# NVIDIA-Merlin/Transformers4Rec

Hardware: AMD Instinct MI355X
Metric: training sessions/sec (XLNet 4x128, 100k items, seq 20, MLM, tied full softmax) + Recall@20 (higher is better)
Workload: dtype f32; 1 GPU; BASELINE.json configs[1]: synthetic schema, item vocab 100k (100001 table rows), d_model 128, 4-layer 4-head XLNet, seq_len 20, per-GPU batch 1024, MLM p=0.15, tied-weight full softmax, Adam, fwd+bwd+gradient exchange+optimizer per step; global_batch=1024, seq_len=20, parallelism=dp1, head_mode=materialize, precision_mode=auto, table_exchange=local, world_size=1, gpu_max_hw_queues=4, extra_streams=0, prefetch=1, preheat_steps=1847

## Files before the change

### transformers4rec_amd/_lib.py

```python
import ctypes
import os
import re

_HERE = os.path.dirname(os.path.abspath(__file__))
LIB_PATH = os.environ.get("T4R_HIP_LIB") or os.path.join(_HERE, "lib", "libt4r_hip.so")
HEADER_PATH = os.path.join(os.path.dirname(_HERE), "include", "t4r_hip.h")
SAMPLING_HEADER_PATH = os.path.join(os.path.dirname(_HERE), "include", "t4r_hip_sampling.h")
FILTER_HEADER_PATH = os.path.join(os.path.dirname(_HERE), "include", "t4r_hip_filter.h")
OPTIM_HEADER_PATH = os.path.join(os.path.dirname(_HERE), "include", "t4r_hip_optim.h")
PRETRAINED_HEADER_PATH = os.path.join(os.path.dirname(_HERE), "include", "t4r_hip_pretrained.h")
ATTN_HEADER_PATH = os.path.join(os.path.dirname(_HERE), "include", "t4r_hip_attn.h")
ROWS_HEADER_PATH = os.path.join(os.path.dirname(_HERE), "include", "t4r_hip_rows.h")
ROWADAM_HEADER_PATH = os.path.join(os.path.dirname(_HERE), "include", "t4r_hip_rowadam.h")
CONTPROJ_HEADER_PATH = os.path.join(os.path.dirname(_HERE), "include", "t4r_hip_contproj.h")
ROWCLIP_HEADER_PATH = os.path.join(os.path.dirname(_HERE), "include", "t4r_hip_rowclip.h")

_P, _I, _L, _F, _Q = ctypes.c_void_p, ctypes.c_int, ctypes.c_long, ctypes.c_float, ctypes.c_ulonglong
_C = {"p": _P, "i": _I, "l": _L, "f": _F, "Q": _Q}

_SIGS = {
    "t4r_abi_version": ("i", ""),
    "t4r_last_error": ("s", ""),
    "t4r_ragged_max_len": ("i", "ppip"),
    "t4r_ragged_to_padded": ("i", "ppppiii"),
    "t4r_ragged_gather_to_padded": ("i", "pppp" + "p" + "iii"),
    "t4r_seq_features_fwd": ("i", "pippppppiiiiiiipppp"),
    "t4r_embedding_bwd": ("i", "pppp" + "liiilii"),
    "t4r_sort_ids_ws_bytes": ("l", "l"),
    "t4r_sort_ids": ("i", "pp" + "lli" + "ppp" + "l"),
    "t4r_sort_ids_multi_ws_bytes": ("l", "li"),
    "t4r_sort_ids_multi": ("i", "ppilpp" + "ppp" + "l"),
    "t4r_embedding_bwd_sorted_ws_floats": ("l", "li"),
    "t4r_embedding_bwd_sorted": ("i", "ppppp" + "liiili" + "p"),
    "t4r_embedding_bag_fwd": ("i", "pp" + "li" + "pp" + "llii" + "p" + "li" + "p"),
    "t4r_embedding_bag_bwd_rows": ("i", "pp" + "lii" + "p" + "llii" + "p"),
    "t4r_apply_mask_fwd": ("i", "ppppiiii"),
    "t4r_apply_mask_bwd": ("i", "ppppiiii" + "p"),
    "t4r_apply_mask_bwd_ws_floats": ("l", "iii"),
    "t4r_apply_mask_bwd_to": ("i", "pppppiiii" + "p"),
    "t4r_mul": ("i", "ppppl"),
    "t4r_soft_embedding_fwd": ("i", "pppppppp" + "liif"),
    "t4r_soft_embedding_bwd": ("i", "pppppppppppp" + "liiiif" + "p"),
    "t4r_soft_embedding_bwd_ws_floats": ("l", "lii"),
    "t4r_mask_targets": ("i", "ppiiil" + "ppp" + "fQQ" + "ppp"),
    "t4r_compact_labels": ("i", "pppiil" + "pppp"),
    "t4r_gather_rows": ("i", "ppppii"),
    "t4r_scatter_rows_add": ("i", "ppppii"),
    "t4r_scatter_rows_dense": ("i", "pppippli"),
    "t4r_last_positions": ("i", "ppiiiilp"),
    "t4r_gemm_f32": ("i", "piiiiif" + "plplpl" + "pipl" + "iii" + "lll" + "fQQ"),
    "t4r_gemm_splitk_sink_begin": ("v", "pl"),
    "t4r_gemm_splitk_sink_flush": ("i", "p"),
    "t4r_gemm_splitk_sink_end": ("v", ""),
    "t4r_gemm_splitk_sink_bypassed": ("i", ""),
    "t4r_mha_fwd": ("i", "pppplplp" + "iiiii" + "fQQ" + "p"),
    "t4r_mha_bwd": ("i", "pppplpplppppl" + "iiiii" + "fQQ" + "p"),
    "t4r_add_pos_fwd": ("i", "ppppp" + "iii"),
    "t4r_add_pos_bwd": ("i", "ppp" + "iii"),
    "t4r_dropout_ctr_hi": ("Q", "Qii"),
    "t4r_dropout": ("i", "pppp" + "llfQQ"),
    "t4r_set_precision": ("v", "i"),
    "t4r_get_precision": ("i", ""),
    "t4r_gemm_softmax_grad_f32": ("i", "piiiif" + "plpppf" + "plpl" + "ii"),
    "t4r_set_tok_gemm_min_rows": ("v", "i"),
    "t4r_get_tok_gemm_min_rows": ("i", ""),
    "t4r_head_split_supported": ("i", "i"),
    "t4r_head_split_fwd_products": ("i", ""),
    "t4r_head_split_ws_bytes": ("l", "iii"),
    "t4r_head_split_prepare": ("i", "ppl" + "iii" + "p"),
    "t4r_head_split_fdx_supported": ("i", "i"),
    "t4r_head_split_logits_ce_dx": ("i", "pp" + "plpl" + "pl" + "pppp" + "plp" + "iii" + "ff" + "p"),
    "t4r_head_note_dw_form": ("i", "p"),
    "t4r_head_split_logits": ("i", "ppplpl" + "iiif" + "p"),
    "t4r_head_split_logits_ce": ("i", "ppplpl" + "pppp" + "iiiff" + "p"),
    "t4r_head_split_dw": ("i", "ppplpppf" + "pl" + "iiiii" + "fi" + "p"),
    "t4r_head_split_dx": ("i", "ppplpppf" + "plpl" + "iiiii" + "fi" + "p"),
    "t4r_head_split_recompute_supported": ("i", "i"),
    "t4r_head_split_prepare_rc": ("i", "ppl" + "iii" + "p"),
    "t4r_head_split_ce": ("i", "ppplpppp" + "iiiff" + "p"),
    "t4r_head_split_dw_rc": ("i", "ppplpppf" + "pl" + "iiifi" + "p"),
    "t4r_head_split_dx_rc": ("i", "ppplplpppf" + "pl" + "iiifi" + "p"),
    "t4r_add_layernorm_fwd": ("i", "pppppppp" + "iif" + "fQQ"),
    "t4r_add_layernorm_bwd": ("i", "pppppppppppp" + "iii" + "fQQ"),
    "t4r_colreduce_ws_floats": ("l", "li"),
    "t4r_act_bwd_bias": ("i", "pppppp" + "lii" + "fQQ"),
    "t4r_colsum": ("i", "pppp" + "lil"),
    "t4r_session_lengths": ("i", "pp" + "iiii" + "p"),
    "t4r_xlnet_attn_fwd": ("i", "ppppppppp" + "iiii" + "ifQQ" + "p"),
    "t4r_xlnet_attn_bwd_ws_floats": ("l", "iiii"),
    "t4r_xlnet_attn_bwd": ("i", "p" * 17 + "iiii" + "ifQQ" + "p"),
    "t4r_xlnet_fused_supported": ("i", "i"),
    "t4r_xlnet_fused_products": ("i", ""),
    "t4r_xlnet_ff_bwd_part_floats": ("l", "li"),
    "t4r_xlnet_layer_planes_floats": ("l", "i"),
    "t4r_xlnet_layer_prepare": ("i", "ppip"),
    "t4r_xlnet_qkv_proj": ("i", "pppp" + "li"),
    "t4r_xlnet_kr_proj": ("i", "pppp" + "li"),
    "t4r_xlnet_oproj_ln": ("i", "p" + "ppppp" + "pppp" + "liff" + "QQ"),
    "t4r_xlnet_ln1_bwd_part_floats": ("l", "li"),
    "t4r_xlnet_ln1_bwd": ("i", "p" + "ppppppp" + "pppppp" + "lif" + "QQ"),
    "t4r_xlnet_dh": ("i", "pppp" + "li"),
    "t4r_xlnet_set_cu_budget": ("v", "i"),
    "t4r_xlnet_get_cu_budget": ("i", ""),
    "t4r_device_cus": ("i", ""),
    "t4r_experimental_build": ("i", ""),
    "t4r_xlnet_attn_block_supported": ("i", "iii"),
    "t4r_xlnet_attn_block_fwd": ("i", "ppppp" + "l" + "pppp" + "ppppppp" + "iiii" + "ffQQQ" + "p"),
    "t4r_xlnet_layer_bwd_defer": ("v", "i"),
    "t4r_xlnet_layer_ws_offsets": ("i", "iiiii" + "pp"),
    "t4r_xlnet_stack_prepare": ("i", "ppiip" + "plp"),
    "t4r_xlnet_stack_pos_dropout": ("v", "fQQlp"),
    "t4r_xlnet_stack_prepared": ("v", "i"),
    "t4r_xlnet_layer_bwd_join": ("i", "p"),
    "t4r_xlnet_ff_planes_floats": ("l", "i"),
    "t4r_xlnet_ff_prepare": ("i", "ppppip"),
    "t4r_xlnet_ff_fwd": ("i", "p" + "pppppp" + "pppppp" + "iiff" + "QQQ"),
    "t4r_xlnet_ff_bwd": ("i", "p" + "pppppppp" + "pppppppp" + "iif" + "QQQ"),
    "t4r_xlnet_layer_ws_floats": ("l", "iiiii"),
    "t4r_xlnet_layer_bwd_ws_floats": ("l", "iiiii"),
    "t4r_xlnet_layer_fwd": ("i", "pppppp" + "iiiif" + "fQQi" + "pp"),
    "t4r_xlnet_layer_bwd": ("i", "ppppppppp" + "iiiif" + "fQQi" + "pp"),
    "t4r_softmax_ce_fwd": ("i", "pppppp" + "iilf"),
    "t4r_softmax_ce_bwd": ("i", "pppppp" + "iilf"),
    "t4r_linear_softmax_ce_chunk_floats": ("l", "ii"),
    "t4r_linear_softmax_ce_fwd": ("i", "pplpl" + "p" + "iiiffi" + "ppppp"),
    "t4r_linear_softmax_ce_bwd": ("i", "pplpl" + "ppp" + "iiiffi" + "pplpl"),
    "t4r_sampled_logits_fwd": ("i", "ppppppp" + "iiif" + "p"),
    "t4r_log_uniform_sample": ("i", "pp" + "ill" + "QQ"),
    "t4r_sampled_logits_bwd": ("i", "ppppppppp" + "iiif"),
    "t4r_sampled_logits_bwd_rows": ("i", "ppppppppp" + "iiif"),
    "t4r_topk": ("i", "pp" + "iili" + "pp"),
    "t4r_rank_of_target_f32": ("i", "p" + "iiif" + "pl" + "pl" + "ppp"),
    "t4r_item_topk_ws_bytes": ("l", "iiii"),
    "t4r_item_topk_f32": ("i", "p" + "iiif" + "pl" + "pl" + "i" + "pp" + "pl" + "p"),
    "t4r_item_table_image_ld": ("i", "i"),
    "t4r_item_topk_h16_supported": ("i", "i"),
    "t4r_item_table_pack_h16": ("i", "p" + "pl" + "iii" + "pl"),
    "t4r_item_scores_h16": ("i", "p" + "iiif" + "pl" + "pl" + "i" + "pl" + "pl"),
    "t4r_item_topk_h16_ws_bytes": ("l", "iiii"),
    "t4r_item_topk_h16": ("i", "p" + "iiif" + "pl" + "pl" + "i" + "i" + "pp" + "pl" + "p"),
    "t4r_item_eval_h16_ws_bytes": ("l", "iii"),
    "t4r_item_eval_h16": ("i", "p" + "iiif" + "pl" + "pl" + "i" + "p" + "pppp" + "pl"),
    "t4r_swap_noise_ws_bytes": ("l", "l"),
    "t4r_swap_noise": ("i", "ppp" + "il" + "pllf" + "pp" + "QQ" + "pl"),
    "t4r_copy_cols": ("i", "pp" + "li" + "p" + "ili"),
    "t4r_seq_sum_cols": ("i", "pp" + "li" + "p" + "ili"),
    "t4r_adam_step": ("i", "ppppp" + "li" + "ffffff" + "i"),
    "t4r_adam_step_amax": ("i", "ppppp" + "li" + "ffffff" + "i" + "llp"),
    "t4r_head_split_w_amax_hint": ("v", "ppi"),
}

_SIGS_SAMPLING = {
    "t4r_gumbel_add_f32": ("i", "pp" + "iill" + "i" + "QQ"),
    "t4r_gumbel_argmax_f32": ("i", "pp" + "iill" + "QQ" + "pp"),
    "t4r_item_sample_ws_bytes": ("l", "iiii"),
    "t4r_item_sample_f32": ("i", "p" + "iiif" + "pl" + "pl" + "i" + "pp" + "pl" + "p" + "lQQ"),
    "t4r_item_sample_h16_ws_bytes": ("l", "iiii"),
    "t4r_item_sample_h16": ("i", "p" + "iiif" + "pl" + "pl" + "i" + "i" + "pp" + "pl" + "p" + "lQQ"),
}

_FILT = "ppil"
_SIGS_FILTER = {
    "t4r_item_allow_words": ("l", "i"),
    "t4r_item_allow_pack": ("i", "ppip"),
    "t4r_item_mask_f32": ("i", "pp" + "iili" + _FILT),
    "t4r_item_topk_filtered_f32": ("i", _SIGS["t4r_item_topk_f32"][1] + _FILT),
    "t4r_item_topk_filtered_h16": ("i", _SIGS["t4r_item_topk_h16"][1] + _FILT),
    "t4r_item_sample_filtered_f32": ("i", _SIGS_SAMPLING["t4r_item_sample_f32"][1] + _FILT),
    "t4r_item_sample_filtered_h16": ("i", _SIGS_SAMPLING["t4r_item_sample_h16"][1] + _FILT),
}

_SIGS_OPTIM = {
    "t4r_grad_sumsq_parts": ("l", "l"),
    "t4r_grad_sumsq": ("i", "pplp"),
    "t4r_grad_clip_coef": ("i", "ppiffp"),
    "t4r_adamw_step": ("i", "ppppp" + "li" + "fffff" + "if" + "i" + "p" + "llp"),
}

_PP = "pipllpli"
_SIGS_PRETRAINED = {
    "t4r_pretrained_proj_ws_bytes": ("l", "ii"),
    "t4r_pretrained_proj_fwd": ("i", _PP + "ppppfii" + "pli" + "pppp"),
    "t4r_pretrained_proj_bwd_ws_floats": ("l", "lii"),
    "t4r_pretrained_proj_bwd": ("i", _PP + "pli" + "ppp" + "ii" + "ppppp"),
}

_SIGS_ATTN = {
    "t4r_xlnet_attn_block_fwd_prob": ("i", "ppppp" + "l" + "pppp" + "pppppppp" + "iiii" + "ffQQQ" + "p"),
    "t4r_xlnet_attn_bwd_prob": ("i", "p" * 16 + "iiii" + "ifQQ"),
}

_SIGS_ROWS = {
    "t4r_xlnet_ff_fwd_rows": ("i", _SIGS["t4r_xlnet_ff_fwd"][1] + "pi"),
    "t4r_xlnet_ff_bwd_rows": ("i", _SIGS["t4r_xlnet_ff_bwd"][1] + "pip"),
    "t4r_xlnet_ln1_bwd_rows": ("i", "p" + "ppppppp" + "ppp" + "ppp" + "lif" + "QQ" + "pi"),
    "t4r_xlnet_layer_fwd_rows": ("i", _SIGS["t4r_xlnet_layer_fwd"][1] + "pi"),
    "t4r_xlnet_layer_bwd_rows": ("i", _SIGS["t4r_xlnet_layer_bwd"][1] + "pi"),
}

_SIGS_ROWADAM = {
    "t4r_row_adam_ws_bytes": ("l", "li"),
    "t4r_row_adam_step": ("i", "pppp" + "li" + "ppp" + "lli" + "fffff" + "if" + "pl"),
}

_CP = "pp" + "liii" + "pp"
_SIGS_CONTPROJ = {
    "t4r_cont_proj_supported": ("i", "ii"),
    "t4r_cont_proj_bwd_ws_floats": ("l", "lii"),
    "t4r_cont_proj_fwd": ("i", "p" + _CP + "p"),
    "t4r_cont_proj_bwd": ("i", "p" + "pli" + _CP + "pppp"),
}

_SIGS_ROWCLIP = {
    "t4r_row_grad_sumsq_parts": ("l", "li"),
    "t4r_row_adam_reduce": ("i", "pli" + "ppp" + "ll" + "pl" + "p"),
    "t4r_row_adam_apply": ("i", "pppp" + "li" + "li" + "fffff" + "if" + "p" + "pl"),
}

_lib = None


class T4RHipError(RuntimeError):
    pass


def _declared(path):
    with open(path) as f:
        text = re.sub(r"/\*.*?\*/", "", f.read(), flags=re.S)
    return sorted(set(re.findall(r"\b(t4r_\w+)\s*\(", text)))


def header_symbols():
    return _declared(HEADER_PATH)


def sampling_header_symbols():
    return _declared(SAMPLING_HEADER_PATH)


def filter_header_symbols():
    return _declared(FILTER_HEADER_PATH)


def optim_header_symbols():
    return _declared(OPTIM_HEADER_PATH)


def pretrained_header_symbols():
    return _declared(PRETRAINED_HEADER_PATH)


def attn_header_symbols():
    return _declared(ATTN_HEADER_PATH)


def rows_header_symbols():
    return _declared(ROWS_HEADER_PATH)


def rowadam_header_symbols():
    return _declared(ROWADAM_HEADER_PATH)


def contproj_header_symbols():
    return _declared(CONTPROJ_HEADER_PATH)


def rowclip_header_symbols():
    return _declared(ROWCLIP_HEADER_PATH)


def load():
    global _lib
    if _lib is not None:
        return _lib
    if not os.path.exists(LIB_PATH):
        raise T4RHipError(
            f"{LIB_PATH} not found: the HIP extension is not built "
            "(run `python -m transformers4rec_amd.build`). There is no CPU fallback.")
    lib = ctypes.CDLL(LIB_PATH)
    for name, (ret, args) in (list(_SIGS.items()) + list(_SIGS_SAMPLING.items()) + list(_SIGS_FILTER.items()) + list(_SIGS_OPTIM.items())
                              + list(_SIGS_PRETRAINED.items()) + list(_SIGS_ATTN.items()) + list(_SIGS_ROWS.items()) + list(_SIGS_ROWADAM.items())
                              + list(_SIGS_CONTPROJ.items()) + list(_SIGS_ROWCLIP.items())):
        fn = getattr(lib, name)
        fn.restype = ctypes.c_char_p if ret == "s" else (None if ret == "v" else _C[ret])
        fn.argtypes = [_C[a] for a in args]
    _lib = lib
    return lib


def check(rc, what):
    if rc != 0:
        msg = load().t4r_last_error()
        raise T4RHipError(f"{what} failed (rc={rc}): {msg.decode() if msg else ''}")


def call(name, *args):
    rc = getattr(load(), name)(*args)
    if rc != 0:
        check(rc, name)


def ptr_array(ptrs):
    arr = (ctypes.c_void_p * len(ptrs))(*ptrs)
    return ctypes.cast(arr, ctypes.c_void_p), arr


def int_array(vals):
    arr = (ctypes.c_int * len(vals))(*vals)
    return ctypes.cast(arr, ctypes.c_void_p), arr


def long_array(vals):
    arr = (ctypes.c_long * len(vals))(*vals)
    return ctypes.cast(arr, ctypes.c_void_p), arr


def exp_env(name, default=None):
    v = os.environ.get(name)
    if v is None:
        return default
    try:
        return v if load().t4r_experimental_build() else default
    except Exception:
        return default
```

### transformers4rec_amd/csrc/embedding_sorted.hip

```cpp
#include "t4r_common.h"
#include "seg_sum_kernel.h"
#include <hipcub/hipcub.hpp>

static size_t al256(size_t b) { return (b + 255) & ~(size_t)255; }

__global__ __launch_bounds__(256) void emb_keys_kernel(const long* __restrict__ ids, long n, long rows,
                                                        int padding_idx, int* __restrict__ keys,
                                                        int* __restrict__ idx) {
    const long i = (long)blockIdx.x * blockDim.x + threadIdx.x;
    if (i >= n) return;
    const long id = ids[i];
    keys[i] = (id == padding_idx || id < 0 || id >= rows) ? (int)rows : (int)id;
    idx[i] = (int)i;
}

struct SortLayout { size_t keys_in, idx_in, tmp, tmp_bytes, total; };
static SortLayout sort_layout(long n) {
    SortLayout l;
    size_t o = 0;
    auto take = [&](size_t b) { size_t at = o; o += al256(b); return at; };
    l.keys_in = take((size_t)n * 4);
    l.idx_in = take((size_t)n * 4);
    size_t sb = 0;
    (void)hipcub::DeviceRadixSort::SortPairs(nullptr, sb, (int*)nullptr, (int*)nullptr, (int*)nullptr,
                                             (int*)nullptr, (int)n);
    l.tmp_bytes = sb;
    l.tmp = take(sb);
    l.total = o;
    return l;
}

extern "C" long t4r_sort_ids_ws_bytes(long n) { return n <= 0 ? 0 : (long)sort_layout(n).total; }

extern "C" int t4r_sort_ids(void* stream, const long* ids, long n, long rows, int padding_idx,
                            int* keys_sorted, int* perm, void* ws, long ws_bytes) {
    if (n <= 0) return 0;
    T4R_CHECK_ARG(ids && keys_sorted && perm && ws, "sort_ids: null pointer");
    T4R_CHECK_ARG(n < (1L << 31) && rows > 0 && rows < (1L << 31) - 1, "sort_ids: sizes must fit 31 bits");
    const SortLayout l = sort_layout(n);
    T4R_CHECK_ARG(ws_bytes >= (long)l.total, "sort_ids: workspace too small (t4r_sort_ids_ws_bytes)");
    hipStream_t st = (hipStream_t)stream;
    char* w = (char*)ws;
    int* keys_in = (int*)(w + l.keys_in);
    int* idx_in = (int*)(w + l.idx_in);
    hipLaunchKernelGGL(emb_keys_kernel, dim3((unsigned)((n + 255) / 256)), dim3(256), 0, st, ids, n, rows,
                       padding_idx, keys_in, idx_in);
    int end_bit = 1;
    while (end_bit < 31 && (1L << end_bit) <= rows) ++end_bit;
    size_t tb = l.tmp_bytes;
    if (hipcub::DeviceRadixSort::SortPairs(w + l.tmp, tb, keys_in, keys_sorted, idx_in, perm, (int)n, 0, end_bit,
                                           st) != hipSuccess) {
        t4r_set_error("sort_ids: device radix sort failed");
        return -1;
    }
    T4R_LAUNCH_CHECK();
    return 0;
}

constexpr int kSortMaxFeatures = 16;
struct SortMulti { const long* ids[kSortMaxFeatures]; long rows[kSortMaxFeatures]; long off[kSortMaxFeatures]; int pad[kSortMaxFeatures]; int F; long n; };

__global__ __launch_bounds__(256) void emb_keys_multi_kernel(SortMulti p, int* __restrict__ keys, int* __restrict__ idx) {
    const long i = (long)blockIdx.x * blockDim.x + threadIdx.x;
    if (i >= p.n * p.F) return;
    const int f = (int)(i / p.n);
    const long id = p.ids[f][i - f * p.n];
    const long rows = p.rows[f];
    keys[i] = (int)(p.off[f] + ((id == p.pad[f] || id < 0 || id >= rows) ? rows : id));
    idx[i] = (int)i;
}
__global__ __launch_bounds__(256) void emb_keys_multi_fix_kernel(SortMulti p, int* __restrict__ keys, int* __restrict__ perm) {
    const long i = (long)blockIdx.x * blockDim.x + threadIdx.x;
    if (i >= p.n * p.F) return;
    const int f = (int)(i / p.n);
    keys[i] -= (int)p.off[f];
    perm[i] -= (int)(f * p.n);
}

extern "C" long t4r_sort_ids_multi_ws_bytes(long n, int F) { return (n <= 0 || F <= 0) ? 0 : (long)sort_layout(n * F).total; }

extern "C" int t4r_sort_ids_multi(void* stream, const long* const* ids, int F, long n, const long* rows, const int* padding_idx,
                                  int* keys_sorted, int* perm, void* ws, long ws_bytes) {
    if (n <= 0 || F <= 0) return 0;
    T4R_CHECK_ARG(ids && rows && padding_idx && keys_sorted && perm && ws, "sort_ids_multi: null pointer");
    T4R_CHECK_ARG(F <= kSortMaxFeatures, "sort_ids_multi: at most 16 tables per call");
    SortMulti p;
    p.F = F; p.n = n;
    long off = 0;
    for (int f = 0; f < F; ++f) {
        T4R_CHECK_ARG(ids[f] && rows[f] > 0, "sort_ids_multi: null ids or empty table");
        p.ids[f] = ids[f]; p.rows[f] = rows[f]; p.pad[f] = padding_idx[f]; p.off[f] = off;
        off += rows[f] + 1;
    }
    T4R_CHECK_ARG(n * F < (1L << 31) && off < (1L << 31) - 1, "sort_ids_multi: sizes must fit 31 bits");
    const SortLayout l = sort_layout(n * F);
    T4R_CHECK_ARG(ws_bytes >= (long)l.total, "sort_ids_multi: workspace too small (t4r_sort_ids_multi_ws_bytes)");
    hipStream_t st = (hipStream_t)stream;
    char* w = (char*)ws;
    int* keys_in = (int*)(w + l.keys_in);
    int* idx_in = (int*)(w + l.idx_in);
    const unsigned grid = (unsigned)((n * F + 255) / 256);
    hipLaunchKernelGGL(emb_keys_multi_kernel, dim3(grid), dim3(256), 0, st, p, keys_in, idx_in);
    int end_bit = 1;
    while (end_bit < 31 && (1L << end_bit) < off) ++end_bit;
    size_t tb = l.tmp_bytes;
    if (hipcub::DeviceRadixSort::SortPairs(w + l.tmp, tb, keys_in, keys_sorted, idx_in, perm, (int)(n * F), 0, end_bit, st) !=
        hipSuccess) {
        t4r_set_error("sort_ids_multi: device radix sort failed");
        return -1;
    }
    hipLaunchKernelGGL(emb_keys_multi_fix_kernel, dim3(grid), dim3(256), 0, st, p, keys_sorted, perm);
    T4R_LAUNCH_CHECK();
    return 0;
}

extern "C" long t4r_embedding_bwd_sorted_ws_floats(long n, int dim) { return seg_ws_floats(n, dim); }

extern "C" int t4r_embedding_bwd_sorted(void* stream, const float* dout, const int* keys_sorted,
                                        const int* perm, float* dtable, long n, int W, int col, int dim,
                                        long rows, int ids_div, float* ws) {
    if (n <= 0) return 0;
    T4R_CHECK_ARG(dout && keys_sorted && perm && dtable && ws, "embedding_bwd_sorted: null pointer");
    T4R_CHECK_ARG(ids_div >= 1 && dim >= 1 && col >= 0 && col + dim <= W, "embedding_bwd_sorted: bad slice");
    T4R_CHECK_ARG(rows < (1L << 31) - 1, "embedding_bwd_sorted: rows must fit 31 bits");
    seg_sum_launch<false>((hipStream_t)stream, dout, keys_sorted, perm, dtable, ws, n, W, col, dim, (int)rows, ids_div);
    T4R_LAUNCH_CHECK();
    return 0;
}
```

### transformers4rec_amd/features.py

```python
import functools
import math
import os
from typing import Dict, Optional

import torch
from torch import nn

from . import ops
from .transformations import TabularDropout, TabularLayerNorm, parse_post, parse_pre
from .masking import MaskSequence, _grad_buf, parse_masking
from .schema import Tags, categorical_cardinalities



def _table_scatter(ctx, name, grad_rows, ids_f, tab, col, dim, padding_idx):
    ids_div = grad_rows.numel() // grad_rows.shape[-1] // ids_f.numel()
    sink = getattr(tab, "_t4r_sparse_sink", None)
    if sink is not None:
        sink.add(tab, ids_f, grad_rows, col, dim, ids_div, padding_idx)
        return
    srt = ctx.sorted_ids.get(name)
    if srt is None:
        srt = ops.sort_ids(ids_f, tab.shape[0], padding_idx)
    ops.embedding_bwd_sorted(grad_rows, srt[0], srt[1], _grad_buf(tab), col, dim, ids_div)


def _sort_ids_forward(ids, rows, padding_idx):
    return ops.sort_ids(ids, rows, padding_idx)


def _sort_ids_forward_multi(ids_list, rows_list, padding_idx):
    return ops.sort_ids_multi(ids_list, rows_list, [padding_idx] * len(ids_list))


class EmbeddingTable(nn.Module):

    def __init__(self, num_embeddings, embedding_dim, padding_idx=None, std=0.05):
        super().__init__()
        self.num_embeddings, self.embedding_dim, self.padding_idx = num_embeddings, embedding_dim, padding_idx
        self.weight = nn.Parameter(torch.empty(num_embeddings, embedding_dim))
        nn.init.normal_(self.weight, mean=0.0, std=std)

    def extra_repr(self):
        return f"{self.num_embeddings}, {self.embedding_dim}, padding_idx={self.padding_idx}"


class _Linear(nn.Module):

    def __init__(self, in_features, out_features, bias=True):
        super().__init__()
        self.in_features, self.out_features = in_features, out_features
        self.weight = nn.Parameter(torch.empty(out_features, in_features))
        self.bias = nn.Parameter(torch.empty(out_features)) if bias else None
        nn.init.kaiming_uniform_(self.weight, a=math.sqrt(5))
        if bias:
            bound = 1 / math.sqrt(in_features) if in_features > 0 else 0
            nn.init.uniform_(self.bias, -bound, bound)


class _LayerNormParams(nn.Module):
    def __init__(self, dim, eps=1e-5):
        super().__init__()
        self.eps = eps
        self.weight = nn.Parameter(torch.ones(dim))
        self.bias = nn.Parameter(torch.zeros(dim))


class SoftEmbedding(nn.Module):

    def __init__(self, num_embeddings, embeddings_dim):
        super().__init__()
        self.embedding_table = EmbeddingTable(num_embeddings, embeddings_dim)
        self.projection_layer = _Linear(1, num_embeddings)


class SequenceEmbeddingFeatures(nn.Module):

    def __init__(self, table_sizes: Dict[str, tuple], item_id: Optional[str] = None, padding_idx: int = 0,
                 pre=None, post=None):
        super().__init__()
        self.item_id = item_id
        self.padding_idx = padding_idx
        self.embedding_tables = nn.ModuleDict(
            {n: EmbeddingTable(v, d, padding_idx=padding_idx) for n, (v, d) in table_sizes.items()})
        self.item_seq = None
        self._pre = parse_pre(pre)
        self._post = parse_post(post, {n: d for n, (v, d) in table_sizes.items()})

    @property
    def pre(self):
        return self._pre

    @property
    def post(self):
        return self._post

    @property
    def item_embedding_table(self):
        assert self.item_id is not None
        return self.embedding_tables[self.item_id]

    def item_ids(self, inputs):
        return inputs[self.item_id]


class TableConfig:

    def __init__(self, vocabulary_size: int, dim: int, initializer=None, combiner: str = "mean", name: Optional[str] = None):
        if not isinstance(vocabulary_size, int) or vocabulary_size < 1:
            raise ValueError("Invalid vocabulary_size {}.".format(vocabulary_size))
        if not isinstance(dim, int) or dim < 1:
            raise ValueError("Invalid dim {}.".format(dim))
        if combiner not in ("mean", "sum", "sqrtn"):
            raise ValueError("Invalid combiner {}".format(combiner))
        if initializer is not None and not callable(initializer):
            raise ValueError("initializer must be callable if specified.")
        self.vocabulary_size, self.dim, self.combiner, self.name = vocabulary_size, dim, combiner, name
        self.initializer = functools.partial(nn.init.normal_, mean=0.0, std=0.05) if initializer is None else initializer

    def __repr__(self):
        return (f"TableConfig(vocabulary_size={self.vocabulary_size!r}, dim={self.dim!r}, "
                f"combiner={self.combiner!r}, name={self.name!r})")


class FeatureConfig:

    def __init__(self, table: TableConfig, max_sequence_length: int = 0, name: Optional[str] = None):
        self.table, self.max_sequence_length, self.name = table, max_sequence_length, name


class _BagTable(nn.Module):

    def __init__(self, num_embeddings, embedding_dim, mode="mean", initializer=None):
        super().__init__()
        self.num_embeddings, self.embedding_dim, self.mode = num_embeddings, embedding_dim, mode
        self.weight = nn.Parameter(torch.empty(num_embeddings, embedding_dim))
        nn.init.normal_(self.weight, mean=0.0, std=0.05)
        if initializer is not None:
            initializer(self.weight)

    def extra_repr(self):
        return f"{self.num_embeddings}, {self.embedding_dim}, mode={self.mode!r}"


class _EmbeddingBagsFn(torch.autograd.Function):

    @staticmethod
    def forward(ctx, anchor, tables, lookups, concat, err):
        B = lookups[0][1].numel() if lookups[0][1] is not None else lookups[0][0].shape[0]
        cols, c = [], 0
        for t in tables:
            cols.append(c)
            c += t.shape[1] if concat else 0
        wide = torch.empty((B, c), device=anchor.device, dtype=torch.float32) if concat else None
        outs, saved = [], []
        for t, (vals, offs, comb), col in zip(tables, lookups, cols):
            vals = vals.contiguous()
            offs = None if offs is None else offs.contiguous()
            outs.append(ops.embedding_bag_fwd(t.detach(), vals, offs, comb, out=wide, col=col, err_flag=err))
            saved.append((vals, offs, comb, 0 if offs is not None else vals.numel() // max(vals.shape[0], 1), col))
        ctx.tables, ctx.saved, ctx.concat = tables, saved, concat
        return (wide,) if concat else tuple(outs)

    @staticmethod
    def backward(ctx, *douts):
        for i, (tab, (vals, offs, comb, fixed_k, col)) in enumerate(zip(ctx.tables, ctx.saved)):
            dout = douts[0] if ctx.concat else douts[i]
            if dout is None:
                continue
            rows = ops.embedding_bag_bwd_rows(dout.contiguous(), vals.numel(), tab.shape[1], offs, fixed_k, comb, col=col)
            ids = vals.view(-1)
            sink = getattr(tab, "_t4r_sparse_sink", None)
            if sink is not None:
                sink.add_rows(tab, ids, rows, padding_idx=-1)
            else:
                ops.scatter_rows_sorted(_grad_buf(tab), ids, rows, padding_idx=-1)
        return None, None, None, None, None


class EmbeddingFeatures(nn.Module):

    def __init__(self, feature_config: Dict[str, FeatureConfig], item_id: Optional[str] = None, pre=None, post=None,
                 aggregation: Optional[str] = None, schema=None):
        super().__init__()
        if pre is not None or post is not None:
# ... 847 lines not shown
```

### transformers4rec_amd/ops.py

```python
import ctypes

import torch

from . import _lib
from ._lib import call, int_array, long_array, ptr_array

EPI_NONE, EPI_BIAS, EPI_BIAS_GELU, EPI_BIAS_RELU, EPI_BIAS_RESID = 0, 1, 2, 3, 4
AGG = {"concat": 0, "element-wise-sum": 1, "element-wise-sum-item-multi": 2}
MASK_NONE, MASK_MLM, MASK_CLM, MASK_CLM_INFER = 0, 1, 2, 3
MLM_TRAIN, MLM_EVAL_LAST, MLM_EVAL_ALL, MLM_INFER, CLM_TRAIN, CLM_LAST, CLM_INFER = range(7)


_GPU_OK = False


def _stream():
    global _GPU_OK
    if not _GPU_OK:
        if not torch.cuda.is_available():
            raise _lib.T4RHipError("no GPU visible to torch: the HIP path cannot run and there is no CPU path")
        _GPU_OK = True
    return torch.cuda.current_stream().cuda_stream


# ... 226 lines not shown
    return bool(_lib.load().t4r_head_split_recompute_supported(int(D)))


def head_split_ce(ws, x, W, labels, alpha=1.0, label_smoothing=0.0):
    N, D = x.shape
    V = W.shape[0]
    dev = x.device
    loss_rows = torch.empty(N, device=dev, dtype=torch.float32)
    lse = torch.empty(N, device=dev, dtype=torch.float32)
    loss = torch.empty((), device=dev, dtype=torch.float32)
    call("t4r_head_split_prepare_rc", _stream(), _chk(x, torch.float32), x.stride(0), N, D, int(V), ws.data_ptr())
    call("t4r_head_split_ce", _stream(), ws.data_ptr(), _chk(W, torch.float32), W.stride(0), _chk(labels, torch.int64),
         loss_rows.data_ptr(), lse.data_ptr(), loss.data_ptr(), N, V, D, float(alpha), float(label_smoothing), _note(ws))
    return loss, loss_rows, lse


def head_split_dw_rc(ws, W, lse, labels, grad_out, out, alpha=1.0, label_smoothing=0.0, accumulate=True):
    N = lse.shape[0]
    V, D = W.shape
    call("t4r_head_split_dw_rc", _stream(), ws.data_ptr(), _chk(W, torch.float32), W.stride(0), _chk(lse, torch.float32),
         _chk(labels, torch.int64), _p(grad_out), float(label_smoothing), out.data_ptr(), out.stride(0), N, V, D, float(alpha),
         int(accumulate), _note(ws))
    return out


def head_split_dx_rc(ws, x, W, lse, labels, grad_out, alpha=1.0, label_smoothing=0.0, out=None, accumulate=False):
    N, D = x.shape
    V = W.shape[0]
    if out is None:
        out = torch.empty((N, D), device=x.device, dtype=torch.float32)
    call("t4r_head_split_dx_rc", _stream(), ws.data_ptr(), _chk(x, torch.float32), x.stride(0), _chk(W, torch.float32), W.stride(0),
         _chk(lse, torch.float32), _chk(labels, torch.int64), _p(grad_out), float(label_smoothing), out.data_ptr(), out.stride(0),
         N, V, D, float(alpha), int(accumulate), _note(ws))
    return out


SITE_INPUT, SITE_POS, SITE_PROB, SITE_ATTN_OUT, SITE_FF_ACT, SITE_FF_OUT, SITE_FINAL = range(7)
SITE_GUMBEL = 7
LAYER_FUSE_FINAL = 0x100
LAYER_FUSE_INPUT = 0x200
NO_DROP = (0.0, 0, 0)


def dropout_ctr_hi(offset, layer, site):
    return _lib.load().t4r_dropout_ctr_hi(int(offset), int(layer), int(site))


def dropout(x, p, seed, ctr_hi, n_total=None, want_mask=False, out=None):
    n_src = x.numel()
    n = n_src if n_total is None else n_total
    if out is None:
        out = torch.empty(n, device=x.device, dtype=torch.float32)
    mask = torch.empty(n, device=x.device, dtype=torch.uint8) if want_mask else None
    call("t4r_dropout", _stream(), _chk(x, torch.float32), out.data_ptr(), _p(mask), n, n_src, float(p),
         int(seed), int(ctr_hi))
    return (out, mask) if want_mask else out


def add_layernorm_fwd(a, b, gamma, beta, eps, drop=NO_DROP):
    rows, D = a.shape[0], a.shape[1]
    y = torch.empty_like(a)
    mean = torch.empty(rows, device=a.device, dtype=torch.float32)
    rstd = torch.empty_like(mean)
    call("t4r_add_layernorm_fwd", _stream(), _chk(a, torch.float32), _p(b, torch.float32),
         _chk(gamma), _chk(beta), y.data_ptr(), mean.data_ptr(), rstd.data_ptr(), rows, D, float(eps),
         float(drop[0]), int(drop[1]), int(drop[2]))
    return y, mean, rstd


def add_layernorm_bwd(a, b, gamma, mean, rstd, dy, dgamma, dbeta, dx=None, accumulate_dx=False,
                      drop=NO_DROP):
    rows, D = a.shape
    if dx is None:
        dx = torch.empty_like(a)
    dxa = torch.empty_like(a) if drop[0] > 0 else None
    ws = _colred_ws(rows, 2 * D, a.device)
    call("t4r_add_layernorm_bwd", _stream(), _chk(a), _p(b), _chk(gamma), _chk(mean), _chk(rstd),
         _chk(dy), dx.data_ptr(), _p(dxa), _p(dgamma), _p(dbeta), ws.data_ptr(), rows, D,
         int(accumulate_dx), float(drop[0]), int(drop[1]), int(drop[2]))
    return dx if dxa is None else (dx, dxa)


def _colred_ws(rows, ncols, device):
    return torch.empty(_lib.load().t4r_colreduce_ws_floats(rows, ncols), device=device, dtype=torch.float32)


def act_bwd_bias(dact, pre, dbias, mode, out=None, drop=NO_DROP):
    rows, N = dact.shape
    out = dact if out is None else out
    ws = None if dbias is None else _colred_ws(rows, N, dact.device)
    call("t4r_act_bwd_bias", _stream(), _chk(dact), _chk(pre), out.data_ptr(), _p(dbias), _p(ws), rows, N,
         mode, float(drop[0]), int(drop[1]), int(drop[2]))
    return out


def colsum_(x, out):
    ws = _colred_ws(x.shape[0], x.shape[1], x.device)
    call("t4r_colsum", _stream(), _chk(x), _chk(out), ws.data_ptr(), x.shape[0], x.shape[1], x.stride(0))
    return out


def ragged_to_padded(values, offsets, L):
    rows = offsets.numel() - 1
    out = torch.empty((rows, L), device=values.device, dtype=values.dtype)
    if values.dtype not in (torch.int64, torch.float32):
        raise TypeError("ragged_to_padded: int64 or float32 values")
    call("t4r_ragged_to_padded", _stream(), _chk(values), _chk(offsets, torch.int64), out.data_ptr(),
         rows, L, values.element_size())
    return out


def ragged_gather_to_padded(values, offsets, row_ids, L):
    rows = row_ids.numel()
    if values.dtype not in (torch.int64, torch.float32):
        raise TypeError("ragged_gather_to_padded: int64 or float32 values")
    scalar = offsets is None
    out = torch.empty((rows,) if scalar else (rows, L), device=values.device, dtype=values.dtype)
    call("t4r_ragged_gather_to_padded", _stream(), _chk(values), _p(offsets, torch.int64),
         _chk(row_ids, torch.int64), out.data_ptr(), rows, 1 if scalar else L, values.element_size())
    return out


def ragged_max_len(offsets):
    out = torch.empty(1, device=offsets.device, dtype=torch.int32)
    call("t4r_ragged_max_len", _stream(), _chk(offsets, torch.int64), offsets.numel() - 1, out.data_ptr())
    return out


def seq_features_fwd(feats, agg, B, L_in, L_out, W, item_feat=-1, mask_mode=MASK_NONE, mask=None,
                     masked_emb=None, err_flag=None):
    n = len(feats)
    dev = feats[0]["input"].device
    out = torch.empty((B, L_out, W), device=dev, dtype=torch.float32)
    kinds, _k = int_array([f["kind"] for f in feats])
    inputs, _i = ptr_array([_chk(f["input"]) for f in feats])
    tables, _t = ptr_array([0 if f.get("table") is None else _chk(f["table"], torch.float32) for f in feats])
    dims, _d = int_array([f["dim"] for f in feats])
    cols, _c = int_array([f.get("col", 0) for f in feats])
    rows, _r = long_array([f.get("rows", 0) for f in feats])
    call("t4r_seq_features_fwd", _stream(), n, kinds, inputs, tables, dims, cols, rows, AGG[agg] if
         isinstance(agg, str) else agg, item_feat, B, L_in, L_out, W, mask_mode,
         _p(mask), _p(masked_emb), out.data_ptr(), _p(err_flag))
    return out


def embedding_bwd(dout, ids, d_table, col, dim, padding_idx=0):
    W = dout.shape[-1]
    ntok = dout.numel() // W
    ids_div = ntok // ids.numel()
    call("t4r_embedding_bwd", _stream(), _chk(dout, torch.float32), _chk(ids, torch.int64),
         _chk(d_table, torch.float32), ntok, W, col, dim, d_table.shape[0], padding_idx, ids_div)


def sort_ids(ids, rows, padding_idx=0):
    ids = ids.contiguous().view(-1)
    n = ids.numel()
    keys = torch.empty(n, device=ids.device, dtype=torch.int32)
    perm = torch.empty(n, device=ids.device, dtype=torch.int32)
    nb = _lib.load().t4r_sort_ids_ws_bytes(n)
    ws = torch.empty(max(nb, 1), device=ids.device, dtype=torch.uint8)
    call("t4r_sort_ids", _stream(), _chk(ids, torch.int64), n, int(rows), int(padding_idx), keys.data_ptr(),
         perm.data_ptr(), ws.data_ptr(), nb)
    return keys, perm


def sort_ids_multi(ids_list, rows_list, padding_idx_list):
    F = len(ids_list)
    ids_list = [i.contiguous().view(-1) for i in ids_list]
    n = ids_list[0].numel()
    if F > 16 or any(i.numel() != n for i in ids_list):
        return [sort_ids(i, r, p) for i, r, p in zip(ids_list, rows_list, padding_idx_list)]
    dev = ids_list[0].device
    keys = torch.empty(F * n, device=dev, dtype=torch.int32)
    perm = torch.empty(F * n, device=dev, dtype=torch.int32)
    nb = _lib.load().t4r_sort_ids_multi_ws_bytes(n, F)
    ws = torch.empty(max(nb, 1), device=dev, dtype=torch.uint8)
    parr, _k0 = ptr_array([_chk(i, torch.int64) for i in ids_list])
    rows, _k1 = long_array([int(r) for r in rows_list])
    pads, _k2 = int_array([int(p) for p in padding_idx_list])
    call("t4r_sort_ids_multi", _stream(), parr, F, n, rows, pads, keys.data_ptr(), perm.data_ptr(), ws.data_ptr(), nb)
    return [(keys[f * n:(f + 1) * n], perm[f * n:(f + 1) * n]) for f in range(F)]


def embedding_bwd_sorted(dout, keys, perm, d_table, col, dim, ids_div=1):
    W = dout.shape[-1]
    n = keys.numel()
    if dout.numel() != n * ids_div * W:
        raise ValueError("embedding_bwd_sorted: dout rows != lookups * ids_div")
    ws = torch.empty(max(1, _lib.load().t4r_embedding_bwd_sorted_ws_floats(n, dim)), device=dout.device,
                     dtype=torch.float32)
    call("t4r_embedding_bwd_sorted", _stream(), _chk(dout, torch.float32), _chk(keys, torch.int32),
         _chk(perm, torch.int32), _chk(d_table, torch.float32), n, W, col, dim, d_table.shape[0], int(ids_div),
         ws.data_ptr())


BAG_COMBINER = {"sum": 0, "mean": 1, "sqrtn": 2}


def embedding_bag_fwd(table, values, offsets=None, combiner="mean", out=None, col=0, err_flag=None):
    rows, dim = table.shape
    if offsets is None:
        v2 = values.view(values.shape[0], -1)
        n_bags, fixed_k = v2.shape[0], v2.shape[1]
    else:
        n_bags, fixed_k = offsets.numel(), 0
    if out is None:
        out = torch.empty((n_bags, dim), device=table.device, dtype=torch.float32)
    call("t4r_embedding_bag_fwd", _stream(), _chk(table, torch.float32), rows, dim, _chk(values, torch.int64),
         _p(offsets, torch.int64), n_bags, values.numel(), fixed_k, BAG_COMBINER[combiner], out.data_ptr(),
         out.stride(0), col, _p(err_flag))
    return out


def embedding_bag_bwd_rows(dout, n_values, dim, offsets=None, fixed_k=0, combiner="mean", col=0):
    rows = torch.empty((n_values, dim), device=dout.device, dtype=torch.float32)
    n_bags = dout.shape[0]
    call("t4r_embedding_bag_bwd_rows", _stream(), _chk(dout, torch.float32), dout.stride(0), col, dim,
         _p(offsets, torch.int64), n_bags, n_values, fixed_k, BAG_COMBINER[combiner], rows.data_ptr())
    return rows


def swap_noise(x, item_ids, p, pad_token=0, bern=None, perm=None, seed=0, ctr_hi=0):
    if x.dtype not in (torch.int64, torch.float32):
        raise TypeError("swap_noise: int64 ids or fp32 values")
    n = x.numel()
    out = torch.empty_like(x)
    stride = item_ids.shape[1] if x.ndim == item_ids.ndim - 1 else 1
    nb = _lib.load().t4r_swap_noise_ws_bytes(n)
    ws = torch.empty(max(nb, 1), device=x.device, dtype=torch.uint8)
    if bern is not None:
        bern = bern.to(torch.uint8).contiguous()
    call("t4r_swap_noise", _stream(), _chk(x), out.data_ptr(), x.element_size(), n,
         _chk(item_ids, torch.int64), int(pad_token), stride, float(p), _p(bern, torch.uint8),
         _p(perm, torch.int64), int(seed), int(ctr_hi), ws.data_ptr(), nb)
    return out


def copy_cols_out(wide2d, col, dim):
    rows, ldw = wide2d.shape
    out = torch.empty((rows, dim), device=wide2d.device, dtype=torch.float32)
    call("t4r_copy_cols", _stream(), _chk(wide2d, torch.float32), ldw, col, out.data_ptr(), dim, rows, 0)
    return out


def seq_sum_cols(wide2d, col, dim, B, L):
    out = torch.empty((B, dim), device=wide2d.device, dtype=torch.float32)
    call("t4r_seq_sum_cols", _stream(), _chk(wide2d, torch.float32), wide2d.shape[1], col, out.data_ptr(), dim,
         B, L)
    return out


def apply_mask_fwd_(x, mask, memb, mode):
    B, L, H = x.shape
    call("t4r_apply_mask_fwd", _stream(), _chk(x), _chk(mask), _chk(memb), B, L, H, mode)
    return x


def apply_mask_bwd_(dy, mask, d_memb, mode):
    B, L, H = dy.shape
    ws = torch.empty(max(1, _lib.load().t4r_apply_mask_bwd_ws_floats(B, L, H)), device=dy.device, dtype=torch.float32)
    call("t4r_apply_mask_bwd", _stream(), _chk(dy), _chk(mask), _chk(d_memb), B, L, H, mode, ws.data_ptr())
    return dy


def apply_mask_bwd(dy, mask, d_memb, mode):
    B, L, H = dy.shape
    dy = dy.contiguous()
    dx = torch.empty_like(dy)
    ws = torch.empty(max(1, _lib.load().t4r_apply_mask_bwd_ws_floats(B, L, H)), device=dy.device, dtype=torch.float32)
    call("t4r_apply_mask_bwd_to", _stream(), _chk(dy), dx.data_ptr(), _chk(mask), _chk(d_memb), B, L, H, mode, ws.data_ptr())
    return dx


def mul(a, b):
    out = torch.empty_like(a)
    call("t4r_mul", _stream(), _chk(a), _chk(b), out.data_ptr(), a.numel())
    return out


def soft_embedding_fwd(x, proj_w, proj_b, table, ln_w, ln_b, eps=1e-5):
    K, D = table.shape
    out = torch.empty(x.shape + (D,), device=x.device, dtype=torch.float32)
    call("t4r_soft_embedding_fwd", _stream(), _chk(x, torch.float32), _chk(proj_w), _chk(proj_b),
         _chk(table), _p(ln_w), _p(ln_b), out.data_ptr(), x.numel(), K, D, float(eps))
    return out


def soft_embedding_bwd(dout, x, proj_w, proj_b, table, ln_w, d_proj_w, d_proj_b, d_table, d_ln_w,
                       d_ln_b, col, eps=1e-5):
    K, D = table.shape
    W = dout.shape[-1]
    ws = torch.empty(max(1, _lib.load().t4r_soft_embedding_bwd_ws_floats(x.numel(), K, D)), device=dout.device, dtype=torch.float32)
    call("t4r_soft_embedding_bwd", _stream(), _chk(dout), _chk(x), _chk(proj_w), _chk(proj_b),
         _chk(table), _p(ln_w), _chk(d_proj_w), _chk(d_proj_b), _chk(d_table), _p(d_ln_w), _p(d_ln_b),
         x.numel(), W, col, K, D, float(eps), ws.data_ptr())


def mask_targets(item_ids, mode, padding_idx=0, bern=None, j1=None, j2=None, p=0.15, seed=0,
                 offset=0, want_counts=True):
    B, L = item_ids.shape
    Lout = L + 1 if mode == MLM_INFER else L
    dev = item_ids.device
    mask = torch.empty((B, Lout), device=dev, dtype=torch.bool)
    labels = torch.empty((B, Lout), device=dev, dtype=torch.int64)
    counts = torch.empty(B, device=dev, dtype=torch.int32) if want_counts else None
    if bern is not None:
        bern = bern.to(torch.uint8) if bern.dtype != torch.uint8 else bern
    call("t4r_mask_targets", _stream(), _chk(item_ids, torch.int64), B, L, mode, padding_idx,
         _p(bern), _p(j1, torch.int64), _p(j2, torch.int64), float(p), int(seed), int(offset),
         mask.data_ptr(), labels.data_ptr(), _p(counts))
    return mask, labels, counts


def compact_labels(labels, counts, padding_idx=0):
    B, L = labels.shape
    dev = labels.device
    row_off = torch.empty(B, device=dev, dtype=torch.int32)
    n = torch.empty(1, device=dev, dtype=torch.int32)
    pos = torch.empty(B * L, device=dev, dtype=torch.int32)
    lab = torch.empty(B * L, device=dev, dtype=torch.int64)
    call("t4r_compact_labels", _stream(), _chk(labels, torch.int64), _chk(counts, torch.int32), B, L,
         padding_idx, row_off.data_ptr(), n.data_ptr(), pos.data_ptr(), lab.data_ptr())
    return n, pos, lab


def gather_rows(x2d, pos, n):
    D = x2d.shape[1]
    out = torch.empty((n, D), device=x2d.device, dtype=torch.float32)
    call("t4r_gather_rows", _stream(), _chk(x2d, torch.float32), _chk(pos, torch.int32), out.data_ptr(), n, D)
    return out


def scatter_rows_add_(dout, pos, dx2d):
# ... 1003 lines not shown
```

Baseline: 432,400 sessions/s.

## Replace hipcub radix sort with bitonic chunk sort plus merge-rank placement for small inputs

For sort inputs up to about 80k ids, packs each key and index into a 64-bit word and bitonic-sorts chunks of 1024 or 2048 in shared memory. A second kernel then finds each element's final position by binary-searching every sorted chunk and summing the ranks, then scatters the key and permutation. This avoids the multi-pass hipcub radix sort and its several launches for the batch of 1024x20 ids. The cost is a rank search that grows with the number of chunks, and words needing the 8-byte alignment of the existing workspace; the library path stays available as a fallback.

```diff
diff --git a/include/t4r_hip_step.h b/include/t4r_hip_step.h
--- /dev/null
+++ b/include/t4r_hip_step.h
@@ -0,0 +1,20 @@
+#ifndef T4R_HIP_STEP_H
+#define T4R_HIP_STEP_H
+
+#ifdef __cplusplus
+extern "C" {
+#endif
+
+long t4r_sort_ids_small_limit(void);
+int t4r_sort_ids_small_chunk(void);
+long t4r_sort_ids_small_chunk_switch(void);
+
+int t4r_sort_ids_library(void* stream, const long* ids, long n, long rows, int padding_idx, int* keys_sorted, int* perm,
+                         void* ws, long ws_bytes);
+int t4r_sort_ids_multi_library(void* stream, const long* const* ids, int F, long n, const long* rows, const int* padding_idx,
+                               int* keys_sorted, int* perm, void* ws, long ws_bytes);
+
+#ifdef __cplusplus
+}
+#endif
+#endif
diff --git a/transformers4rec_amd/_lib.py b/transformers4rec_amd/_lib.py
--- a/transformers4rec_amd/_lib.py
+++ b/transformers4rec_amd/_lib.py
@@ -14,6 +14,7 @@
 ROWADAM_HEADER_PATH = os.path.join(os.path.dirname(_HERE), "include", "t4r_hip_rowadam.h")
 CONTPROJ_HEADER_PATH = os.path.join(os.path.dirname(_HERE), "include", "t4r_hip_contproj.h")
 ROWCLIP_HEADER_PATH = os.path.join(os.path.dirname(_HERE), "include", "t4r_hip_rowclip.h")
+STEP_HEADER_PATH = os.path.join(os.path.dirname(_HERE), "include", "t4r_hip_step.h")
 
 _P, _I, _L, _F, _Q = ctypes.c_void_p, ctypes.c_int, ctypes.c_long, ctypes.c_float, ctypes.c_ulonglong
 _C = {"p": _P, "i": _I, "l": _L, "f": _F, "Q": _Q}
@@ -217,6 +218,14 @@
     "t4r_row_adam_apply": ("i", "pppp" + "li" + "li" + "fffff" + "if" + "p" + "pl"),
 }
 
+_SIGS_STEP = {
+    "t4r_sort_ids_small_limit": ("l", ""),
+    "t4r_sort_ids_small_chunk": ("i", ""),
+    "t4r_sort_ids_small_chunk_switch": ("l", ""),
+    "t4r_sort_ids_library": ("i", _SIGS["t4r_sort_ids"][1]),
+    "t4r_sort_ids_multi_library": ("i", _SIGS["t4r_sort_ids_multi"][1]),
+}
+
 _lib = None
 
 
@@ -268,6 +277,10 @@
 
 def rowclip_header_symbols():
     return _declared(ROWCLIP_HEADER_PATH)
+
+
+def step_header_symbols():
+    return _declared(STEP_HEADER_PATH)
 
 
 def load():
@@ -281,7 +294,7 @@
     lib = ctypes.CDLL(LIB_PATH)
     for name, (ret, args) in (list(_SIGS.items()) + list(_SIGS_SAMPLING.items()) + list(_SIGS_FILTER.items()) + list(_SIGS_OPTIM.items())
                               + list(_SIGS_PRETRAINED.items()) + list(_SIGS_ATTN.items()) + list(_SIGS_ROWS.items()) + list(_SIGS_ROWADAM.items())
-                              + list(_SIGS_CONTPROJ.items()) + list(_SIGS_ROWCLIP.items())):
+                              + list(_SIGS_CONTPROJ.items()) + list(_SIGS_ROWCLIP.items()) + list(_SIGS_STEP.items())):
         fn = getattr(lib, name)
         fn.restype = ctypes.c_char_p if ret == "s" else (None if ret == "v" else _C[ret])
         fn.argtypes = [_C[a] for a in args]
diff --git a/transformers4rec_amd/csrc/embedding_sorted.hip b/transformers4rec_amd/csrc/embedding_sorted.hip
--- a/transformers4rec_amd/csrc/embedding_sorted.hip
+++ b/transformers4rec_amd/csrc/embedding_sorted.hip
@@ -32,14 +32,148 @@
 
 extern "C" long t4r_sort_ids_ws_bytes(long n) { return n <= 0 ? 0 : (long)sort_layout(n).total; }
 
-extern "C" int t4r_sort_ids(void* stream, const long* ids, long n, long rows, int padding_idx,
-                            int* keys_sorted, int* perm, void* ws, long ws_bytes) {
+constexpr int kSortMaxFeatures = 16;
+struct SortMulti { const long* ids[kSortMaxFeatures]; long rows[kSortMaxFeatures]; long off[kSortMaxFeatures]; int pad[kSortMaxFeatures]; int F; long n; };
+constexpr int kSortChunk = 1024;
+constexpr long kSortChunkSwitch = 32768;
+constexpr int kSortFlight = 4;
+constexpr long kSortSmallLimit = 81920;
+typedef unsigned long long sort_word;
+
+__device__ __forceinline__ sort_word sort_word_of(const SortMulti& p, int g) {
+    const int f = (int)(g / p.n);
+    const long id = p.ids[f][g - f * p.n];
+    const long rows = p.rows[f];
+    const long key = p.off[f] + ((id == p.pad[f] || id < 0 || id >= rows) ? rows : id);
+    return ((sort_word)key << 32) | (sort_word)(unsigned)g;
+}
+
+template <int CH>
+__global__ __launch_bounds__(CH / 2) void sort_chunks_kernel(SortMulti p, sort_word* __restrict__ words) {
+    __shared__ sort_word s[CH];
+    const int tid = threadIdx.x;
+    const long total = p.n * p.F;
+    const long base = (long)blockIdx.x * CH;
+#pragma unroll
+    for (int h = 0; h < 2; ++h) {
+        const long g = base + tid + h * (CH / 2);
+        s[tid + h * (CH / 2)] = g < total ? sort_word_of(p, (int)g) : ~(sort_word)0;
+    }
+    __syncthreads();
+#pragma unroll
+    for (int k = 2; k <= CH; k <<= 1) {
+#pragma unroll
+        for (int j = k >> 1; j > 0; j >>= 1) {
+            const int l = tid & (j - 1);
+            const int i = ((tid - l) << 1) + l;
+            const sort_word a = s[i], b = s[i + j];
+            const bool up = (i & k) == 0;
+            if ((a > b) == up) { s[i] = b; s[i + j] = a; }
+            if (j >= 128 || (j == 1 && k >= 128 && k < CH)) {
+                __syncthreads();
+            } else {
+                __builtin_amdgcn_fence(__ATOMIC_RELEASE, "wavefront");
+                __builtin_amdgcn_wave_barrier();
+                __builtin_amdgcn_fence(__ATOMIC_ACQUIRE, "wavefront");
+            }
+        }
+    }
+    __syncthreads();
+#pragma unroll
+    for (int h = 0; h < 2; ++h) {
+        const long g = base + tid + h * (CH / 2);
+        if (g < total) words[g] = s[tid + h * (CH / 2)];
+    }
+}
+
+template <int CH>
+__global__ __launch_bounds__(1024) void sort_place_kernel(SortMulti p, const sort_word* __restrict__ words, int* __restrict__ keys_sorted,
+                                                          int* __restrict__ perm) {
+    __shared__ int part[16][64];
+    const long total = p.n * p.F;
+    const int lane = threadIdx.x & 63, w = __builtin_amdgcn_readfirstlane(threadIdx.x >> 6), W = blockDim.x >> 6;
+    const long at = (long)blockIdx.x * 64 + lane;
+    const bool live = at < total;
+    const sort_word x = words[live ? at : total - 1];
+    const int nchunks = (int)((total + CH - 1) / CH);
+    int rank = 0;
+    for (int c0 = w; c0 < nchunks; c0 += W * kSortFlight) {
+        int len[kSortFlight], cnt[kSortFlight];
+#pragma unroll
+        for (int q = 0; q < kSortFlight; ++q) {
+            const int c = c0 + q * W;
+            const long left = total - (long)c * CH;
+            len[q] = c < nchunks ? (int)(left < CH ? left : CH) : 0;
+            cnt[q] = 0;
+        }
+#pragma unroll 1
+        for (int step = CH; step > 0; step >>= 1) {
+            sort_word v[kSortFlight];
+#pragma unroll
+            for (int q = 0; q < kSortFlight; ++q) {
+                const int e = cnt[q] + step;
+                v[q] = words[e <= len[q] ? (long)(c0 + q * W) * CH + e - 1 : 0];
+            }
+#pragma unroll
+            for (int q = 0; q < kSortFlight; ++q) {
+                const int e = cnt[q] + step;
+                if (e <= len[q] && v[q] < x) cnt[q] = e;
+            }
+        }
+#pragma unroll
+        for (int q = 0; q < kSortFlight; ++q) rank += cnt[q];
+    }
+    part[w][lane] = rank;
+    __syncthreads();
+    if (w != 0 || !live) return;
+    long pos = 0;
+    for (int u = 0; u < W; ++u) pos += part[u][lane];
+    const int g = (int)(unsigned)x;
+    const int f = (int)(g / p.n);
+    keys_sorted[pos] = (int)((long)(x >> 32) - p.off[f]);
+    perm[pos] = (int)(g - f * p.n);
+}
+
+template <int CH>
+static void sort_small_launch(hipStream_t st, const SortMulti& p, sort_word* words, int* keys_sorted, int* perm) {
+    const long total = p.n * p.F;
+    const long nchunks = (total + CH - 1) / CH;
+    long W = (nchunks + kSortFlight - 1) / kSortFlight;
+    W = W > 16 ? 16 : W;
+    hipLaunchKernelGGL(sort_chunks_kernel<CH>, dim3((unsigned)nchunks), dim3(CH / 2), 0, st, p, words);
+    hipLaunchKernelGGL(sort_place_kernel<CH>, dim3((unsigned)((total + 63) / 64)), dim3((unsigned)(64 * W)), 0, st, p, words, keys_sorted, perm);
+}
+
+static bool sort_small(hipStream_t st, const SortMulti& p, int* keys_sorted, int* perm, void* ws, size_t ws_total) {
+    const long total = p.n * p.F;
+    if (total > kSortSmallLimit) return false;
+    const uintptr_t a = ((uintptr_t)ws + 7) & ~(uintptr_t)7;
+    if ((a - (uintptr_t)ws) + (size_t)total * sizeof(sort_word) > ws_total) return false;
+    if (total <= kSortChunkSwitch) sort_small_launch<kSortChunk>(st, p, (sort_word*)a, keys_sorted, perm);
+    else sort_small_launch<2 * kSortChunk>(st, p, (sort_word*)a, keys_sorted, perm);
+    return true;
+}
+
+extern "C" long t4r_sort_ids_small_limit(void) { return kSortSmallLimit; }
+extern "C" int t4r_sort_ids_small_chunk(void) { return kSortChunk; }
+extern "C" long t4r_sort_ids_small_chunk_switch(void) { return kSortChunkSwitch; }
+
+static int sort_ids_impl(void* stream, const long* ids, long n, long rows, int padding_idx, int* keys_sorted, int* perm, void* ws,
+                         long ws_bytes, bool small) {
     if (n <= 0) return 0;
     T4R_CHECK_ARG(ids && keys_sorted && perm && ws, "sort_ids: null pointer");
     T4R_CHECK_ARG(n < (1L << 31) && rows > 0 && rows < (1L << 31) - 1, "sort_ids: sizes must fit 31 bits");
     const SortLayout l = sort_layout(n);
     T4R_CHECK_ARG(ws_bytes >= (long)l.total, "sort_ids: workspace too small (t4r_sort_ids_ws_bytes)");
     hipStream_t st = (hipStream_t)stream;
+    if (small && n <= kSortSmallLimit) {
+        SortMulti p;
+        p.F = 1; p.n = n; p.ids[0] = ids; p.rows[0] = rows; p.pad[0] = padding_idx; p.off[0] = 0;
+        if (sort_small(st, p, keys_sorted, perm, ws, l.total)) {
+            T4R_LAUNCH_CHECK();
+            return 0;
+        }
+    }
     char* w = (char*)ws;
     int* keys_in = (int*)(w + l.keys_in);
     int* idx_in = (int*)(w + l.idx_in);
@@ -56,9 +190,14 @@
     T4R_LAUNCH_CHECK();
     return 0;
 }
-
-constexpr int kSortMaxFeatures = 16;
-struct SortMulti { const long* ids[kSortMaxFeatures]; long rows[kSortMaxFeatures]; long off[kSortMaxFeatures]; int pad[kSortMaxFeatures]; int F; long n; };
+extern "C" int t4r_sort_ids(void* stream, const long* ids, long n, long rows, int padding_idx,
+                            int* keys_sorted, int* perm, void* ws, long ws_bytes) {
+    return sort_ids_impl(stream, ids, n, rows, padding_idx, keys_sorted, perm, ws, ws_bytes, true);
+}
+extern "C" int t4r_sort_ids_library(void* stream, const long* ids, long n, long rows, int padding_idx,
+                                    int* keys_sorted, int* perm, void* ws, long ws_bytes) {
+    return sort_ids_impl(stream, ids, n, rows, padding_idx, keys_sorted, perm, ws, ws_bytes, false);
+}
 
 __global__ __launch_bounds__(256) void emb_keys_multi_kernel(SortMulti p, int* __restrict__ keys, int* __restrict__ idx) {
     const long i = (long)blockIdx.x * blockDim.x + threadIdx.x;
@@ -79,8 +218,8 @@
 
 extern "C" long t4r_sort_ids_multi_ws_bytes(long n, int F) { return (n <= 0 || F <= 0) ? 0 : (long)sort_layout(n * F).total; }
 
-extern "C" int t4r_sort_ids_multi(void* stream, const long* const* ids, int F, long n, const long* rows, const int* padding_idx,
-                                  int* keys_sorted, int* perm, void* ws, long ws_bytes) {
+static int sort_ids_multi_impl(void* stream, const long* const* ids, int F, long n, const long* rows, const int* padding_idx,
+                               int* keys_sorted, int* perm, void* ws, long ws_bytes, bool small) {
     if (n <= 0 || F <= 0) return 0;
     T4R_CHECK_ARG(ids && rows && padding_idx && keys_sorted && perm && ws, "sort_ids_multi: null pointer");
     T4R_CHECK_ARG(F <= kSortMaxFeatures, "sort_ids_multi: at most 16 tables per call");
@@ -96,6 +235,10 @@
     const SortLayout l = sort_layout(n * F);
     T4R_CHECK_ARG(ws_bytes >= (long)l.total, "sort_ids_multi: workspace too small (t4r_sort_ids_multi_ws_bytes)");
     hipStream_t st = (hipStream_t)stream;
+    if (small && sort_small(st, p, keys_sorted, perm, ws, l.total)) {
+        T4R_LAUNCH_CHECK();
+        return 0;
+    }
     char* w = (char*)ws;
     int* keys_in = (int*)(w + l.keys_in);
     int* idx_in = (int*)(w + l.idx_in);
@@ -113,6 +256,14 @@
     T4R_LAUNCH_CHECK();
     return 0;
 }
+extern "C" int t4r_sort_ids_multi(void* stream, const long* const* ids, int F, long n, const long* rows, const int* padding_idx,
+                                  int* keys_sorted, int* perm, void* ws, long ws_bytes) {
+    return sort_ids_multi_impl(stream, ids, F, n, rows, padding_idx, keys_sorted, perm, ws, ws_bytes, true);
+}
+extern "C" int t4r_sort_ids_multi_library(void* stream, const long* const* ids, int F, long n, const long* rows,
+                                          const int* padding_idx, int* keys_sorted, int* perm, void* ws, long ws_bytes) {
+    return sort_ids_multi_impl(stream, ids, F, n, rows, padding_idx, keys_sorted, perm, ws, ws_bytes, false);
+}
 
 extern "C" long t4r_embedding_bwd_sorted_ws_floats(long n, int dim) { return seg_ws_floats(n, dim); }
 
diff --git a/transformers4rec_amd/features.py b/transformers4rec_amd/features.py
--- a/transformers4rec_amd/features.py
+++ b/transformers4rec_amd/features.py
@@ -25,12 +25,15 @@
     ops.embedding_bwd_sorted(grad_rows, srt[0], srt[1], _grad_buf(tab), col, dim, ids_div)
 
 
+_SMALL_SORT = True
+
+
 def _sort_ids_forward(ids, rows, padding_idx):
-    return ops.sort_ids(ids, rows, padding_idx)
+    return ops.sort_ids(ids, rows, padding_idx, small=_SMALL_SORT)
 
 
 def _sort_ids_forward_multi(ids_list, rows_list, padding_idx):
-    return ops.sort_ids_multi(ids_list, rows_list, [padding_idx] * len(ids_list))
+    return ops.sort_ids_multi(ids_list, rows_list, [padding_idx] * len(ids_list), small=_SMALL_SORT)
 
 
 class EmbeddingTable(nn.Module):
diff --git a/transformers4rec_amd/ops.py b/transformers4rec_amd/ops.py
--- a/transformers4rec_amd/ops.py
+++ b/transformers4rec_amd/ops.py
@@ -402,24 +402,24 @@
          _chk(d_table, torch.float32), ntok, W, col, dim, d_table.shape[0], padding_idx, ids_div)
 
 
-def sort_ids(ids, rows, padding_idx=0):
+def sort_ids(ids, rows, padding_idx=0, small=True):
     ids = ids.contiguous().view(-1)
     n = ids.numel()
     keys = torch.empty(n, device=ids.device, dtype=torch.int32)
     perm = torch.empty(n, device=ids.device, dtype=torch.int32)
     nb = _lib.load().t4r_sort_ids_ws_bytes(n)
     ws = torch.empty(max(nb, 1), device=ids.device, dtype=torch.uint8)
-    call("t4r_sort_ids", _stream(), _chk(ids, torch.int64), n, int(rows), int(padding_idx), keys.data_ptr(),
-         perm.data_ptr(), ws.data_ptr(), nb)
+    call("t4r_sort_ids" if small else "t4r_sort_ids_library", _stream(), _chk(ids, torch.int64), n, int(rows), int(padding_idx),
+         keys.data_ptr(), perm.data_ptr(), ws.data_ptr(), nb)
     return keys, perm
 
 
-def sort_ids_multi(ids_list, rows_list, padding_idx_list):
+def sort_ids_multi(ids_list, rows_list, padding_idx_list, small=True):
     F = len(ids_list)
     ids_list = [i.contiguous().view(-1) for i in ids_list]
     n = ids_list[0].numel()
     if F > 16 or any(i.numel() != n for i in ids_list):
-        return [sort_ids(i, r, p) for i, r, p in zip(ids_list, rows_list, padding_idx_list)]
+        return [sort_ids(i, r, p, small) for i, r, p in zip(ids_list, rows_list, padding_idx_list)]
     dev = ids_list[0].device
     keys = torch.empty(F * n, device=dev, dtype=torch.int32)
     perm = torch.empty(F * n, device=dev, dtype=torch.int32)
@@ -428,7 +428,7 @@
     parr, _k0 = ptr_array([_chk(i, torch.int64) for i in ids_list])
     rows, _k1 = long_array([int(r) for r in rows_list])
     pads, _k2 = int_array([int(p) for p in padding_idx_list])
-    call("t4r_sort_ids_multi", _stream(), parr, F, n, rows, pads, keys.data_ptr(), perm.data_ptr(), ws.data_ptr(), nb)
+    call("t4r_sort_ids_multi" if small else "t4r_sort_ids_multi_library", _stream(), parr, F, n, rows, pads, keys.data_ptr(), perm.data_ptr(), ws.data_ptr(), nb)
     return [(keys[f * n:(f + 1) * n], perm[f * n:(f + 1) * n]) for f in range(F)]
 
 
```

Measured after the change: 433,700 sessions/s, median of 4. No clear change (+0.3%).
